# radhofan/Fairify

Measured on AMD Instinct MI355X. Metric: % partitions verified + partitions/sec on AC suite at 1/2/4/8 MI355X, higher is better.
Workload: dtype fp32

## Files before the change

fairify_amd/csrc/bindings.cpp:

```cpp
#include <hip/hip_runtime.h>
#include <pybind11/pybind11.h>
#include <pybind11/stl.h>

#include <algorithm>
#include <cmath>
#include <cstring>
#include <cstdint>
#include <stdexcept>
#include <vector>

#include "kwargs.h"
#include "runtime_host.h"

extern "C" int fa_bounds_launch(const NetDesc& net, BoundArgs args, hipStream_t stream);
extern "C" int fa_crown_phase_launch(const NetDesc& net, CrownPhaseArgs a, hipStream_t stream);
extern "C" size_t fa_crown_phase_bytes(const NetDesc& net);
extern "C" int fa_point_try_launch(const NetDesc& net, BoundArgs a, hipStream_t stream);
extern "C" int fa_forward_launch(const NetDesc& net, FwdArgs a, hipStream_t stream);
extern "C" int fa_sim_launch(const NetDesc& net, SimArgs a, hipStream_t stream);
extern "C" int fa_sim_shaped(const NetDesc& net);
extern "C" int fa_rate_launch(const NetDesc& net, RateArgs a, hipStream_t stream);
extern "C" int fa_count_enum_launch(const NetDesc& net, EnumArgs a, hipStream_t stream);
extern "C" int fa_count_rows_launch(CountArgs a, hipStream_t stream);
extern "C" int fa_count_level_launch(CountArgs a, hipStream_t stream);
// ... 213 lines not shown
  a.tau = k.f("tau", 0.f);
  a.osg = k.ptr<const int8_t>("osg");
  a.pgsum = k.ptr<const float>("pgsum");
  a.pgn = k.ptr<const float>("pgn");
  a.fpar = k.ptr<float>("fpar");
  a.fgt = k.ptr<float>("fgt");
  a.fval = k.ptr<double>("fval");
  if ((net.d.dims[0] < 64 && (a.ramask >> net.d.dims[0])) || (a.ramask && (!a.plo || !a.phi)))
    throw std::invalid_argument("beta_level: RA mask beyond the inputs or no x' box");
  return a;
}

PYBIND11_MODULE(_C, m) {
  m.doc() = "fairify_amd CDNA4 (gfx950) kernels";
  py::class_<Net>(m, "Net")
      .def(py::init<const std::vector<int>&, double>())
      .def_readonly("n_params", &Net::n_params)
      .def_readonly("total_floats", &Net::total_floats)
      .def_property_readonly("wperm_off", [](const Net& n) { return n.d.wperm_off; })
      .def_property_readonly("pack_g", [](const Net& n) { return n.d.pack_g; })
      .def_property_readonly("pack_off", [](const Net& n) { return n.d.pack_off; })
      .def_property_readonly("n_hidden", [](const Net& n) { return n.d.n_hidden; })
      .def_property_readonly("n_neurons", [](const Net& n) { return n.d.n_neurons; });

  m.def("bounds", [](const Net& net, py::kwargs kw) {
    Kw k("bounds", kw);
    const int symbolic = k.i("symbolic");
    BoundArgs a = bound_args(k, symbolic ? OUT | FORMS : OUT);
    a.symbolic = symbolic;
    a.G = k.i("G", 0);
    a.dead_out = k.ptr<uint8_t>("dead_out");
    a.fold = k.u64("fold", 0);
    a.phase_in = k.ptr<const int8_t>("phase_in");
    a.infeas = k.ptr<uint8_t>("infeas");
    ckl(fa_bounds_launch(net.d, a, finish(k)), "bounds");
  });

  m.def("crown_phase", [](const Net& net, py::kwargs kw) {
    Kw k("crown_phase", kw);
    CrownPhaseArgs a = row_args<CrownPhaseArgs>(k, OUT | FORMS | LAYERS);
    a.phase = k.ptr<const int8_t>("phase");
    a.infeas = k.ptr<const uint8_t>("infeas");
    a.split = k.need<int>("split");
    a.score = k.need<float>("score");
    a.low = k.ptr<float>("low");
    const int rc = fa_crown_phase_launch(net.d, a, finish(k));
    if (rc != 0) throw std::runtime_error("crown_phase launch failed, code " + std::to_string(rc));
  });

  m.def("relu_fits", [](const Net& net) { return fa_crown_phase_bytes(net.d) > 0; });

  m.def("crown", [](const Net& net, py::kwargs kw) {
    Kw k("crown", kw);
    const BoundArgs a = bound_args(k, OUT | FORMS | LAYERS);
    ckl(fa_crown_launch(net.d, a, finish(k)), "crown");
  });

  m.def("refine", [](const Net& net, py::kwargs kw) {
    Kw k("refine", kw);
    BoundArgs a = bound_args(k, LAYERS);
    a.phase_in = k.ptr<const int8_t>("phase_in");
    a.infeas = k.ptr<uint8_t>("infeas");
    const int rc = fa_refine_launch(net.d, a, finish(k));
    if (rc < -1) throw std::runtime_error("refine launch failed, code " + std::to_string(rc));
    return rc;
  });
  m.def("refine_crown", [](const Net& net, py::kwargs kw) {
    Kw k("refine_crown", kw);
    const BoundArgs a = bound_args(k, OUT | FORMS | LAYERS);
    const int rc = fa_refine_crown_launch(net.d, a, finish(k));
    if (rc < -1) throw std::runtime_error("refine_crown launch failed, code " + std::to_string(rc));
    return rc;
  });
  m.def("backward_bounds", [](const Net& net, py::kwargs kw) {
    Kw k("backward_bounds", kw);
    const BoundArgs a = bound_args(k, OUT | FORMS);
    const int rc = fa_backward_launch(net.d, a, finish(k));
    if (rc < -1) throw std::runtime_error("backward_bounds launch failed, code " + std::to_string(rc));
    return rc;
  });

  m.def("point_bounds", [](const Net& net, py::kwargs kw) {
    Kw k("point_bounds", kw);
    const BoundArgs a = bound_args(k, OUT, "x", "x");
    const hipStream_t stream = finish(k);
    const int rc = fa_point_try_launch(net.d, a, stream);
    if (rc < 0) ckl(-rc, "point_bounds");
    if (rc == 0) ckl(fa_bounds_launch(net.d, a, stream), "point_bounds(ibp)");
  });

  m.def("forward", [](const Net& net, uintptr_t flat, uintptr_t x, int B, uintptr_t dead, uintptr_t out,
                      uintptr_t stream) {
    FwdArgs a{};
    a.flat = P<const float>(flat);
    a.x = P<const float>(x);
    a.B = B;
    a.dead = P<const uint8_t>(dead);
    a.out = P<float>(out);
    ckl(fa_forward_launch(net.d, a, (hipStream_t)stream), "forward");
  });

  m.def("sim", [](const Net& net, py::kwargs kw) {
    Kw k("sim", kw);
    SimArgs a{};
    fill_query(a, k, "too many PA/RA dims");
    fill_samples(a, k, "too many PA/RA dims");
    a.counts = k.need<int>("counts");
    a.found = k.need<uint8_t>("found");
    a.wit_x = k.need<float>("wit_x");
    a.wit_xp = k.need<float>("wit_xp");
    a.z0 = k.ptr<float>("z0");
    a.keys = k.ptr<int>("keys");
    a.split = k.i("split");
    a.regcount = k.i("regcount");
    if (a.split < 1 || (a.split > 1 && !a.keys)) throw std::invalid_argument("sim: split > 1 needs a keys buffer");
    ckl(fa_sim_launch(net.d, a, finish(k)), "sim");
  });
  m.def("sim_shaped", [](const Net& net) { return fa_sim_shaped(net.d) != 0; });

  m.def("rate", [](const Net& net, py::kwargs kw) {
    Kw k("rate", kw);
    RateArgs a{};
    fill_query(a, k, "too many PA/RA dims");
    fill_samples(a, k, "too many PA/RA dims");
    a.E = k.i("E");
    a.flips = k.need<int>("flips");
    a.amb = k.need<int>("amb");
    a.amb_idx = k.need<int>("amb_idx");
    a.split = k.i("split");
    const int rc = fa_rate_launch(net.d, a, finish(k));
    if (rc == -3) throw std::invalid_argument("rate: shape not covered (layer > 160, inputs > 32, V > 32 or E > 32)");
    ckl(rc, "rate");
  });

  m.def("count_enum", [](const Net& net, py::kwargs kw) {
    Kw k("count_enum", kw);
    EnumArgs a{};
    a.flat = k.need<const float>("flat");
    a.lo = k.need<const float>("lo");
    a.hi = k.need<const float>("hi");
    a.L = k.i("L");
    a.V = k.i("V");
    a.npa = dims(k, "pa", a.pa_idx, FA_MAX_PA, "too many PA/RA dims");
    a.values = k.need<const int64_t>("values");
    a.Pp = k.i("Pp");
    a.pairs = k.ptr<const int64_t>("pairs");
    a.nra = dims(k, "ra", a.ra_idx, FA_MAX_RA, "too many PA/RA dims");
    a.tau = k.i("tau");
    a.E = k.i("E");
    a.max_vol = k.i("max_vol");
    a.cert = k.need<int>("cert");
    a.amb = k.need<int>("amb");
    a.amb_idx = k.need<int>("amb_idx");
    a.blocks = k.i("blocks");
    if (a.Pp > 0 && !a.pairs) throw py::type_error("count_enum() missing required keyword argument 'pairs'");
    const int rc = fa_count_enum_launch(net.d, a, finish(k));
    if (rc == -3)
      throw std::invalid_argument(
          "count_enum: shape not covered (layer > 160, inputs > 32, V > 32, E > 32 or leaf volume > 65536)");
    ckl(rc, "count_enum");
  });
  auto count_args = [](Kw& k) {
    CountArgs a{};
    a.N = k.i("N");
    a.n0 = k.i("n0");
    a.V = k.i("V");
    a.npa = dims(k, "pa", a.pa_idx, FA_MAX_PA, "too many PA/RA dims");
// ... 247 lines not shown
```

fairify_amd/csrc/crown.hip:

```cpp
#include <hip/hip_runtime.h>

#include <stdlib.h>

#include <algorithm>
#include <map>
#include <mutex>

#include "args.h"

#define FA_CROWN_MAXW 256
#define FA_CROWN_WAVES 4

__device__ __forceinline__ float fa_gam(int k, float u) {
  const float ku = (float)(k + 2) * u;
  return ku / (1.f - ku) * (1.f + 4.f * u);
}

template <int G>
__device__ __forceinline__ float fa_group_sum(float v) {
#pragma unroll
  for (int off = G / 2; off > 0; off >>= 1) v += __shfl_xor(v, off, 64);
  return v;
}

template <int G>
__global__ void __launch_bounds__(64 * FA_CROWN_WAVES) fa_crown_kernel(NetDesc net, BoundArgs a, int nparams, int WP) {
  extern __shared__ __attribute__((aligned(16))) float smem[];
  constexpr int RPW = 64 / G;
  const int tid = threadIdx.x;
  for (int l = 0; l < net.n_layers; ++l) {
    const int nin = net.dims[l], nout = net.dims[l + 1];
    const float* src = a.flat + net.w_off[l];
    float* dst = smem + net.w_off[l];
    for (int e = tid; e < nin * nout; e += 64 * FA_CROWN_WAVES) {
      const int j = e / nin, i = e - j * nin;
      dst[e] = src[(size_t)i * nout + j];
    }
    for (int e = tid; e < nout; e += 64 * FA_CROWN_WAVES) smem[net.b_off[l] + e] = a.flat[net.b_off[l] + e];
  }
  __syncthreads();
  const int lane = tid & 63;
  const int wave = tid >> 6;
  const int grp = lane / G;
  const int gl = lane % G;
  float* lam = smem + nparams + (wave * RPW + grp) * (4 * WP + 1);
  float* mu = lam + 2 * WP;
  const int L = net.n_layers;
  const int n0 = net.dims[0];
  const int N = net.n_neurons;
  const float u = net.unit;
  const int rows_per_block = FA_CROWN_WAVES * RPW;
  for (int rb = blockIdx.x * rows_per_block; rb < a.R; rb += gridDim.x * rows_per_block) {
    const int r0 = rb + wave * RPW + grp;
    const bool valid = r0 < a.R;
    const int r = valid ? r0 : a.R - 1;
    const int node = a.V > 0 ? r / a.V : r;
    const int v = a.V > 0 ? r - node * a.V : 0;
    const uint8_t* dmask = nullptr;
    if (a.dead_in) dmask = a.dead_in + (size_t)r * net.n_hidden;
    else if (a.dead_part) dmask = a.dead_part + (size_t)a.node_part[node] * net.n_hidden;
    const float* lbr = a.layer_lb + (size_t)r * N;
    const float* ubr = a.layer_ub + (size_t)r * N;
    {
      const int n = net.dims[L - 1];
      const float* W = smem + net.w_off[L - 1];
      for (int i = gl; i < n; i += G) {
        lam[i] = W[i];
        lam[WP + i] = -W[i];
      }
    }
    float c[2], err[2];
    c[0] = smem[net.b_off[L - 1]];
    c[1] = -c[0];
    err[0] = err[1] = 0.f;
    __builtin_amdgcn_wave_barrier();
    for (int l = L - 2; l >= 0; --l) {
      const int n = net.dims[l + 1];
      const int nin = net.dims[l];
      const int off = net.neuron_off[l];
      const float* W = smem + net.w_off[l];
      const float* b = smem + net.b_off[l];
      float cs[2] = {0.f, 0.f}, cm[2] = {0.f, 0.f}, er[2] = {0.f, 0.f};
      for (int j = gl; j < n; j += G) {
        const float lb = lbr[off + j], ub = ubr[off + j];
        const bool dd = ub <= 0.f || (dmask && dmask[off + j]);
        const bool act = !dd && lb >= 0.f;
        const bool unst = !dd && !act;
        const float alpha = ub > -lb ? 1.f : 0.f;
        const float s = unst ? (ub / (ub - lb)) * (1.f + 4.f * u) : 0.f;
        const float zmax = fmaxf(fabsf(lb), fabsf(ub));
        const float bj = b[j];
#pragma unroll
        for (int sg = 0; sg < 2; ++sg) {
          const float lm = lam[sg * WP + j];
          const float slope = act ? 1.f : (dd ? 0.f : (lm >= 0.f ? alpha : s));
          const float m = lm * slope;
// ... 10 lines not shown
      for (int i = gl; i < nin; i += G) {
        float acc0 = 0.f, acc1 = 0.f, mag0 = 0.f, mag1 = 0.f;
        for (int j = 0; j < n; ++j) {
          const float w = W[(size_t)j * nin + i];
          const float m0 = mu[j], m1 = mu[WP + j];
          acc0 = fmaf(w, m0, acc0);
          acc1 = fmaf(w, m1, acc1);
          mag0 = fmaf(fabsf(w), fabsf(m0), mag0);
          mag1 = fmaf(fabsf(w), fabsf(m1), mag1);
        }
        float hm;
        if (l > 0) {
          const int po = net.neuron_off[l - 1];
          hm = fmaxf(ubr[po + i], 0.f);
          if (dmask && dmask[po + i]) hm = 0.f;
        } else {
          float xl = a.lo[(size_t)node * n0 + i], xh = a.hi[(size_t)node * n0 + i];
          if (a.V > 0)
            for (int k = 0; k < a.npa; ++k)
              if (a.pa_idx[k] == i) xl = xh = a.values[v * a.npa + k];
          hm = fmaxf(fabsf(xl), fabsf(xh));
        }
        lam[i] = acc0;
        lam[WP + i] = acc1;
        er[0] += gn * mag0 * hm;
        er[1] += gn * mag1 * hm;
      }
      const float gc = fa_gam(2 * n + 1, u);
#pragma unroll
      for (int sg = 0; sg < 2; ++sg) {
        const float csum = fa_group_sum<G>(cs[sg]);
        const float cmag = fa_group_sum<G>(cm[sg]);
        const float esum = fa_group_sum<G>(er[sg]);
        const float cold = c[sg];
        c[sg] = cold + csum;
        err[sg] += esum + gc * (fabsf(cold) + cmag);
      }
      __builtin_amdgcn_wave_barrier();
    }
    int K = 4 * L + 4;
    for (int l = 0; l < L; ++l) K += 2 * net.dims[l + 1];
    const float gK = fa_gam(K, u);
    const float g0 = fa_gam(n0 + 1, u);
    const float g1 = fa_gam(1, u);
    float low[2];
#pragma unroll
    for (int sg = 0; sg < 2; ++sg) {
      float cp = 0.f, mp = 0.f;
      for (int i = gl; i < n0; i += G) {
        float xl = a.lo[(size_t)node * n0 + i], xh = a.hi[(size_t)node * n0 + i];
        if (a.V > 0)
          for (int k = 0; k < a.npa; ++k)
            if (a.pa_idx[k] == i) xl = xh = a.values[v * a.npa + k];
        const float lm = lam[sg * WP + i];
        cp += fminf(lm * xl, lm * xh);
        mp += fabsf(lm) * fmaxf(fabsf(xl), fabsf(xh));
      }
      const float conc = fa_group_sum<G>(cp) + c[sg];
      const float cmg = fa_group_sum<G>(mp) + fabsf(c[sg]);
      err[sg] *= 1.f + 2.f * gK;
      low[sg] = conc - err[sg] - g0 * cmg - g1 * fabsf(conc);
    }
    if (valid) {
      const float olb = a.out_lb[r], oub = a.out_ub[r];
      const bool useL = low[0] >= olb;
      const bool useU = -low[1] <= oub;
      for (int i = gl; i < n0; i += G) {
        if (useL) a.Lc[(size_t)r * n0 + i] = lam[i];
        if (useU) a.Uc[(size_t)r * n0 + i] = -lam[WP + i];
      }
      if (gl == 0) {
        if (useL) { a.L0[r] = c[0]; a.Le[r] = err[0]; a.out_lb[r] = low[0]; }
        if (useU) { a.U0[r] = -c[1]; a.Ue[r] = err[1]; a.out_ub[r] = -low[1]; }
      }
    }
    __builtin_amdgcn_wave_barrier();
  }
}

struct CrownCfg {
  int w_lds[FA_MAX_LAYERS];
  int b_lds[FA_MAX_LAYERS];
  int floats;
};

#ifndef FA_CROWN_WPE4
#define FA_CROWN_WPE4 3
#endif
#ifndef FA_CROWN_WPE7
#define FA_CROWN_WPE7 2
#endif
template <int TM>
__global__ void __launch_bounds__(256)
__attribute__((amdgpu_waves_per_eu(TM == 4 ? FA_CROWN_WPE4 : (TM == 7 ? FA_CROWN_WPE7 : 1)))) fa_crown_mfma_kernel(NetDesc net, BoundArgs a, CrownCfg cfg) {
  extern __shared__ __attribute__((aligned(16))) float smem[];
  const int tid = threadIdx.x;
  for (int l = 0; l < net.n_layers; ++l) {
    const int nin = net.dims[l], nout = net.dims[l + 1];
    const int tin = (nin + 15) >> 4, tout = (nout + 15) >> 4;
    const float* W = a.flat + net.w_off[l];
    float* dst = smem + cfg.w_lds[l];
    const int tot = tin * tout * 256;
    for (int e = tid; e < tot; e += 256) {
      const int i4 = e & 3, ln = (e >> 2) & 63, tt = e >> 8;
      const int t = tt % tout, ot = tt / tout;
      const int in = 16 * ot + (ln & 15), out = 16 * t + 4 * (ln >> 4) + i4;
      dst[e] = (in < nin && out < nout) ? W[(size_t)in * nout + out] : 0.f;
    }
    for (int e = tid; e < nout; e += 256) smem[cfg.b_lds[l] + e] = a.flat[net.b_off[l] + e];
  }
  __syncthreads();
  const int lane = tid & 63, col = lane & 15, grp = lane >> 4;
  const int wave = tid >> 6;
  const int L = net.n_layers;
  const int n0 = net.dims[0];
  const int N = net.n_neurons;
  const float u = net.unit;
  const int ntile = (a.R + 15) >> 4;
  for (int tile = blockIdx.x * 4 + wave; tile < ntile; tile += gridDim.x * 4) {
    const int r0 = tile * 16 + col;
    const bool valid = r0 < a.R;
    const int r = valid ? r0 : a.R - 1;
    const int node = a.V > 0 ? r / a.V : r;
    const int v = a.V > 0 ? r - node * a.V : 0;
    if (a.skip_status) {
      const int8_t st = a.skip_status[a.skip_part[node]];
      if (!__any(valid && (st == 3 || st == 4))) continue;
    }
    const uint8_t* dmask = nullptr;
    if (a.dead_in) dmask = a.dead_in + (size_t)r * net.n_hidden;
    else if (a.dead_part) dmask = a.dead_part + (size_t)a.node_part[a.part_mod ? node % a.part_mod : node] * net.n_hidden;
    const float* lbr = a.layer_lb + (size_t)r * N;
    const float* ubr = a.layer_ub + (size_t)r * N;
    float lam[2][TM][4];
    {
      const int n = net.dims[L - 1];
      const float* W = a.flat + net.w_off[L - 1];
#pragma unroll
      for (int t = 0; t < TM; ++t)
#pragma unroll
        for (int i = 0; i < 4; ++i) {
          const int j = 16 * t + 4 * grp + i;
          const float w = j < n ? W[j] : 0.f;
          lam[0][t][i] = w;
          lam[1][t][i] = -w;
        }
    }
    float c[2], err[2];
    c[0] = smem[cfg.b_lds[L - 1]];
    c[1] = -c[0];
    err[0] = err[1] = 0.f;
    for (int l = L - 2; l >= 0; --l) {
      const int n = net.dims[l + 1];
      const int nin = net.dims[l];
      const int tout = (n + 15) >> 4, tin = (nin + 15) >> 4;
      const int off = net.neuron_off[l];
      const float* b = smem + cfg.b_lds[l];
      float mu[2][TM][4];
      float cs[2] = {0.f, 0.f}, cm[2] = {0.f, 0.f}, er[2] = {0.f, 0.f};
#pragma unroll
      for (int t = 0; t < TM; ++t)
#pragma unroll
        for (int i = 0; i < 4; ++i) {
          const int j = 16 * t + 4 * grp + i;
          const bool jv = t < tout && j < n;
          const float lb = jv ? lbr[off + j] : 0.f, ub = jv ? ubr[off + j] : 0.f;
          const bool dd = !jv || ub <= 0.f || (dmask && dmask[off + j]);
          const bool act = !dd && lb >= 0.f;
          const bool unst = !dd && !act;
          const float alpha = ub > -lb ? 1.f : 0.f;
          const float sl = unst ? (ub / (ub - lb)) * (1.f + 4.f * u) : 0.f;
          const float zmax = fmaxf(fabsf(lb), fabsf(ub));
          const float bj = jv ? b[j] : 0.f;
#pragma unroll
          for (int sg = 0; sg < 2; ++sg) {
            const float lm = lam[sg][t][i];
            const float slope = act ? 1.f : (dd ? 0.f : (lm >= 0.f ? alpha : sl));
            const float m = lm * slope;
            const bool neg = unst && lm < 0.f;
            const float tt = neg ? -m * lb : 0.f;
            mu[sg][t][i] = m;
            cs[sg] += m * bj + tt;
            cm[sg] += fabsf(m * bj) + fabsf(tt);
            if (neg) er[sg] += 3.f * u * (fabsf(m) * zmax + fabsf(tt));
          }
        }
      float amu[2][TM][4];
#pragma unroll
      for (int t = 0; t < TM; ++t)
#pragma unroll
        for (int i = 0; i < 4; ++i) {
          amu[0][t][i] = fabsf(mu[0][t][i]);
          amu[1][t][i] = fabsf(mu[1][t][i]);
        }
      const float4* wb = reinterpret_cast<const float4*>(smem + cfg.w_lds[l]);
      const float gn = fa_gam(2 * n + 1, u);
#pragma unroll
      for (int ot = 0; ot < TM; ++ot) {
        if (ot >= tin) break;
        f32x4 Z0 = {0.f, 0.f, 0.f, 0.f}, Z1 = Z0, Q0 = Z0, Q1 = Z0;
#pragma unroll
        for (int t = 0; t < TM; ++t) {
          if (t >= tout) break;
          const float4 w4 = wb[(ot * tout + t) * 64 + lane];
          const float wv[4] = {w4.x, w4.y, w4.z, w4.w};
#pragma unroll
          for (int i = 0; i < 4; ++i) {
            const float aw = fabsf(wv[i]);
            Z0 = fa_mfma4(wv[i], mu[0][t][i], Z0);
            Z1 = fa_mfma4(wv[i], mu[1][t][i], Z1);
            Q0 = fa_mfma4(aw, amu[0][t][i], Q0);
            Q1 = fa_mfma4(aw, amu[1][t][i], Q1);
          }
        }
#pragma unroll
        for (int i = 0; i < 4; ++i) {
          const int in = 16 * ot + 4 * grp + i;
          float hm = 0.f;
          if (in < nin) {
            if (l > 0) {
              const int po = net.neuron_off[l - 1];
              hm = fmaxf(ubr[po + in], 0.f);
              if (dmask && dmask[po + in]) hm = 0.f;
            } else {
              float xl = a.lo[(size_t)node * n0 + in], xh = a.hi[(size_t)node * n0 + in];
              if (a.V > 0)
                for (int k = 0; k < a.npa; ++k)
                  if (a.pa_idx[k] == in) xl = xh = a.values[v * a.npa + k];
              hm = fmaxf(fabsf(xl), fabsf(xh));
            }
          }
          lam[0][ot][i] = in < nin ? Z0[i] : 0.f;
          lam[1][ot][i] = in < nin ? Z1[i] : 0.f;
          er[0] += gn * Q0[i] * hm;
          er[1] += gn * Q1[i] * hm;
        }
      }
#pragma unroll
      for (int ot = 0; ot < TM; ++ot)
        if (ot >= tin)
#pragma unroll
          for (int i = 0; i < 4; ++i) lam[0][ot][i] = lam[1][ot][i] = 0.f;
      const float gc = fa_gam(2 * n + 1, u);
#pragma unroll
      for (int sg = 0; sg < 2; ++sg) {
        float csum = cs[sg], cmag = cm[sg], esum = er[sg];
        csum += __shfl_xor(csum, 16); csum += __shfl_xor(csum, 32);
        cmag += __shfl_xor(cmag, 16); cmag += __shfl_xor(cmag, 32);
        esum += __shfl_xor(esum, 16); esum += __shfl_xor(esum, 32);
        const float cold = c[sg];
        c[sg] = cold + csum;
        err[sg] += esum + gc * (fabsf(cold) + cmag);
      }
    }
    int K = 4 * L + 4;
    for (int l = 0; l < L; ++l) K += 2 * net.dims[l + 1];
    const float gK = fa_gam(K, u);
    const float g0 = fa_gam(n0 + 1, u);
    const float g1 = fa_gam(1, u);
    float low[2];
#pragma unroll
    for (int sg = 0; sg < 2; ++sg) {
      float cp = 0.f, mp = 0.f;
#pragma unroll
      for (int t = 0; t < TM; ++t)
#pragma unroll
        for (int i = 0; i < 4; ++i) {
          const int in = 16 * t + 4 * grp + i;
          if (in >= n0) continue;
          float xl = a.lo[(size_t)node * n0 + in], xh = a.hi[(size_t)node * n0 + in];
          if (a.V > 0)
            for (int k = 0; k < a.npa; ++k)
              if (a.pa_idx[k] == in) xl = xh = a.values[v * a.npa + k];
          const float lm = lam[sg][t][i];
          cp += fminf(lm * xl, lm * xh);
          mp += fabsf(lm) * fmaxf(fabsf(xl), fabsf(xh));
        }
      cp += __shfl_xor(cp, 16); cp += __shfl_xor(cp, 32);
      mp += __shfl_xor(mp, 16); mp += __shfl_xor(mp, 32);
      const float conc = cp + c[sg];
      const float cmg = mp + fabsf(c[sg]);
      err[sg] *= 1.f + 2.f * gK;
      low[sg] = conc - err[sg] - g0 * cmg - g1 * fabsf(conc);
    }
    if (valid) {
      const float olb = a.out_lb[r], oub = a.out_ub[r];
      const bool useL = low[0] >= olb;
      const bool useU = -low[1] <= oub;
#pragma unroll
      for (int t = 0; t < TM; ++t)
#pragma unroll
        for (int i = 0; i < 4; ++i) {
          const int in = 16 * t + 4 * grp + i;
          if (in >= n0) continue;
          if (useL) a.Lc[(size_t)r * n0 + in] = lam[0][t][i];
          if (useU) a.Uc[(size_t)r * n0 + in] = -lam[1][t][i];
        }
      if (grp == 0) {
        if (useL) { a.L0[r] = c[0]; a.Le[r] = err[0]; a.out_lb[r] = low[0]; }
        if (useU) { a.U0[r] = -c[1]; a.Ue[r] = err[1]; a.out_ub[r] = -low[1]; }
      }
    }
  }
}

namespace {
typedef void (*CrownMfmaKernel)(NetDesc, BoundArgs, CrownCfg);
CrownMfmaKernel select_crown_mfma(int TM) {
  if (TM <= 1) return fa_crown_mfma_kernel<1>;
  if (TM <= 2) return fa_crown_mfma_kernel<2>;
  if (TM <= 4) return fa_crown_mfma_kernel<4>;
  if (TM <= 7) return fa_crown_mfma_kernel<7>;
  return nullptr;
}

int crown_cus() {
  static int cus = 0;
  static std::once_flag once;
  std::call_once(once, [] {
    int dev = 0;
    if (hipGetDevice(&dev) != hipSuccess ||
        hipDeviceGetAttribute(&cus, hipDeviceAttributeMultiprocessorCount, dev) != hipSuccess || cus <= 0)
      cus = 256;
  });
  return cus;
}

int crown_mfma_try(const NetDesc& net, const BoundArgs& a, hipStream_t stream) {
  static const bool off = [] {
    const char* e = getenv("FAIRIFY_CROWN_MFMA");
    return e && e[0] == '0';
  }();
  if (off) return 0;
  int TM = 1;
  for (int l = 0; l <= net.n_layers; ++l) TM = std::max(TM, (net.dims[l] + 15) / 16);
  CrownMfmaKernel k = select_crown_mfma(TM);
  if (!k) return 0;
  CrownCfg cfg{};
  int offs = 0;
  for (int l = 0; l < net.n_layers; ++l) {
    cfg.w_lds[l] = offs;
    offs += ((net.dims[l] + 15) / 16) * ((net.dims[l + 1] + 15) / 16) * 256;
  }
  for (int l = 0; l < net.n_layers; ++l) {
    cfg.b_lds[l] = offs;
    offs += net.dims[l + 1];
  }
  cfg.floats = (offs + 3) & ~3;
  const size_t bytes = (size_t)cfg.floats * sizeof(float);
  if (bytes > 150 * 1024) return 0;
  static std::mutex mu;
  static std::map<std::pair<const void*, size_t>, int> occ;
  int per_cu = 0;
  {
    std::lock_guard<std::mutex> g(mu);
    const auto key = std::make_pair((const void*)k, bytes);
    auto it = occ.find(key);
    if (it == occ.end()) {
      if (!fa_lds_ok(bytes)) return -4;
      if (hipOccupancyMaxActiveBlocksPerMultiprocessor(&per_cu, k, 256, bytes) != hipSuccess || per_cu <= 0) per_cu = 1;
      occ[key] = per_cu;
    } else {
      per_cu = it->second;
    }
  }
  const long long tiles = (a.R + 15) / 16;
  long long blocks = (tiles + 3) / 4;
  const long long cap = (long long)crown_cus() * per_cu;
  if (blocks > cap) blocks = cap;
  hipLaunchKernelGGL(k, dim3((unsigned)blocks), dim3(256), bytes, stream, net, a, cfg);
  const hipError_t e = hipGetLastError();
  return e == hipSuccess ? 1 : -(int)e;
}
}

extern "C" int fa_crown_launch(const NetDesc& net, BoundArgs a, hipStream_t stream) {
  if (a.R <= 0) return 0;
  if (!a.layer_lb || !a.layer_ub || !a.Lc || !a.Uc) return -2;
  {
    const int rc = crown_mfma_try(net, a, stream);
    if (rc == 1) return 0;
    if (rc < 0) return -3;
  }
  int wmax = 1;
  for (int l = 0; l <= net.n_layers; ++l) {
    if (net.dims[l] > FA_CROWN_MAXW) return -1;
    if (l > 0) wmax = std::max(wmax, net.dims[l]);
  }
  int G = 4;
  while (G < wmax && G < 64) G *= 2;
  const int WP = (std::max(wmax, net.dims[0]) + 3) & ~3;
  int nparams = 0;
  for (int l = 0; l < net.n_layers; ++l) nparams = net.b_off[l] + net.dims[l + 1];
  const int rows_per_block = FA_CROWN_WAVES * (64 / G);
  const size_t bytes = ((size_t)nparams + (size_t)rows_per_block * (4 * WP + 1)) * sizeof(float);
  if (bytes > 160 * 1024) return -1;
  typedef void (*K)(NetDesc, BoundArgs, int, int);
  K k = G == 4 ? fa_crown_kernel<4> : G == 8 ? fa_crown_kernel<8> : G == 16 ? fa_crown_kernel<16>
      : G == 32 ? fa_crown_kernel<32> : fa_crown_kernel<64>;
  if (!fa_lds_ok(bytes)) return -3;
  const int blocks = (int)std::min<long long>(((long long)a.R + rows_per_block - 1) / rows_per_block, 256LL * 8);
  hipLaunchKernelGGL(k, dim3(blocks), dim3(64 * FA_CROWN_WAVES), bytes, stream, net, a, nparams, WP);
  return (int)hipGetLastError();
}

FA_LDS_REGISTER(FA_LDS_K(fa_crown_mfma_kernel<1>), FA_LDS_K(fa_crown_mfma_kernel<2>), FA_LDS_K(fa_crown_mfma_kernel<4>),
                FA_LDS_K(fa_crown_mfma_kernel<7>), FA_LDS_K(fa_crown_kernel<4>), FA_LDS_K(fa_crown_kernel<8>),
                FA_LDS_K(fa_crown_kernel<16>), FA_LDS_K(fa_crown_kernel<32>), FA_LDS_K(fa_crown_kernel<64>));
```

fairify_amd/csrc/points.hip:

```cpp
#include <hip/hip_runtime.h>

#include <algorithm>
#include <map>
#include <mutex>

#include "pointfwd.h"

template <int TM>
__global__ void __launch_bounds__(FA_THREADS) __attribute__((amdgpu_waves_per_eu(TM == 7 ? 2 : 1))) fa_point_kernel(NetDesc net, BoundArgs a, PointCfg cfg) {
  extern __shared__ __attribute__((aligned(16))) float smem[];
  const int tid = threadIdx.x;
  {
    const float4* src = reinterpret_cast<const float4*>(a.flat + net.wperm_off);
    float4* dst = reinterpret_cast<float4*>(smem);
    for (int e = tid; e < (net.wperm_floats >> 2); e += FA_THREADS) dst[e] = src[e];
    for (int l = 0; l < net.n_layers; ++l) {
      const int n_out = net.dims[l + 1];
      const float* b = a.flat + net.wperm_off + cfg.b_lds[l];
      for (int j = tid; j < ((n_out + 15) & ~15); j += FA_THREADS) smem[cfg.bp_lds[l] + j] = j < n_out ? b[j] : 0.f;
    }
  }
  __syncthreads();
  const int lane = tid & 63, col = lane & 15, grp = lane >> 4;
  const int wave = tid >> 6, nw = FA_THREADS / 64;
  const int n0 = net.dims[0];
  const int tin0 = (n0 + 15) >> 4;
  const float g0 = net.g_fwd[0];
  const int ntile = (a.R + 15) >> 4;
  for (int tile = blockIdx.x * nw + wave; tile < ntile; tile += gridDim.x * nw) {
    const int p0 = tile * 16;
    const int p = p0 + col;
    if (a.row_open && !__any(p < a.R && a.row_open[p % a.open_mod])) continue;
    float HA[TM][4], EA[TM][4], HB[TM][4], EB[TM][4];
#pragma unroll
    for (int t = 0; t < TM; ++t) {
      if (t >= tin0) break;
#pragma unroll
      for (int i = 0; i < 4; ++i) {
        const int k = 16 * t + 4 * grp + i;
        const float x = (k < n0 && p < a.R) ? a.lo[(size_t)p * n0 + k] : 0.f;
        HA[t][i] = x;
        EA[t][i] = g0 * fabsf(x);
      }
    }
    for (int l = 0; l < net.n_layers; ++l) {
      if (l & 1) fa_point_layer<TM>(net, a, cfg, smem, l, p0, lane, HB, EB, HA, EA);
      else fa_point_layer<TM>(net, a, cfg, smem, l, p0, lane, HA, EA, HB, EB);
    }
  }
}

namespace {
typedef void (*PointKernel)(NetDesc, BoundArgs, PointCfg);

PointKernel select_point(int TM) {
  if (TM <= 1) return fa_point_kernel<1>;
  if (TM <= 2) return fa_point_kernel<2>;
  if (TM <= 4) return fa_point_kernel<4>;
  if (TM <= 7) return fa_point_kernel<7>;
  if (TM <= 10) return fa_point_kernel<10>;
  return nullptr;
}

int point_cus() {
  static int cus = 0;
  static std::once_flag once;
  std::call_once(once, [] {
    int dev = 0;
    if (hipGetDevice(&dev) != hipSuccess ||
        hipDeviceGetAttribute(&cus, hipDeviceAttributeMultiprocessorCount, dev) != hipSuccess || cus <= 0)
      cus = 256;
  });
  return cus;
}
}

extern "C" int fa_point_try_launch(const NetDesc& net, BoundArgs a, hipStream_t stream) {
  if (a.R <= 0) return 1;
  int TM = 1;
  for (int l = 0; l <= net.n_layers; ++l) TM = std::max(TM, (net.dims[l] + 15) / 16);
  PointKernel k = select_point(TM);
  if (!k) return 0;
  PointCfg cfg{};
  int off = 0;
  for (int l = 0; l < net.n_layers; ++l) {
    cfg.w_lds[l] = off;
    off += ((net.dims[l] + 15) / 16) * ((net.dims[l + 1] + 15) / 16) * 256;
  }
  for (int l = 0; l < net.n_layers; ++l) {
    cfg.b_lds[l] = off;
    off += net.dims[l + 1];
  }
  if (((off + 3) & ~3) != net.wperm_floats) return -1;
  if ((size_t)net.wperm_floats * sizeof(float) > 150 * 1024) return 0;
// ... 34 lines not shown
```

Baseline: 268,100.

## Specialize CROWN MFMA kernel on compile-time network shapes and dead-mask presence

Adds templated CROWN kernels specialized for known network shapes (AC suite architectures), unrolling layers at compile time with constexpr offsets, cached input-box registers, and a no-mask variant that drops dead-neuron loads. It also copies pre-permuted weights into LDS with float4 when available, and lets the point-bounds kernel exit early when no rows in the block are open. The aim is to cut register pressure, index arithmetic and redundant global loads in the hot backward pass, at the cost of many more kernel instantiations and longer compile time. Floating-point contraction is disabled and some arithmetic is rewritten as explicit fmaf, which keeps the rounding-error bounds sound.

```diff
diff --git a/fairify_amd/csrc/bindings.cpp b/fairify_amd/csrc/bindings.cpp
--- a/fairify_amd/csrc/bindings.cpp
+++ b/fairify_amd/csrc/bindings.cpp
@@ -319,7 +319,10 @@
 
   m.def("point_bounds", [](const Net& net, py::kwargs kw) {
     Kw k("point_bounds", kw);
-    const BoundArgs a = bound_args(k, OUT, "x", "x");
+    BoundArgs a = bound_args(k, OUT, "x", "x");
+    a.row_open = k.ptr<const uint8_t>("row_open");
+    a.open_mod = k.i("open_mod", 0);
+    if (a.row_open && a.open_mod <= 0) throw std::invalid_argument("point_bounds: row_open needs open_mod > 0");
     const hipStream_t stream = finish(k);
     const int rc = fa_point_try_launch(net.d, a, stream);
     if (rc < 0) ckl(-rc, "point_bounds");
diff --git a/fairify_amd/csrc/crown.hip b/fairify_amd/csrc/crown.hip
--- a/fairify_amd/csrc/crown.hip
+++ b/fairify_amd/csrc/crown.hip
@@ -12,6 +12,7 @@
 #define FA_CROWN_WAVES 4
 
 __device__ __forceinline__ float fa_gam(int k, float u) {
+#pragma clang fp contract(off)
   const float ku = (float)(k + 2) * u;
   return ku / (1.f - ku) * (1.f + 4.f * u);
 }
@@ -188,7 +189,203 @@
   int w_lds[FA_MAX_LAYERS];
   int b_lds[FA_MAX_LAYERS];
   int floats;
+  int wfloats;
+  int wcopy;
 };
+
+template <class S>
+struct CrownLay {
+  __host__ __device__ static constexpr int tiles(int l) { return (S::dim(l) + 15) / 16; }
+  __host__ __device__ static constexpr int w_lds(int l) {
+    int o = 0;
+    for (int k = 0; k < l; ++k) o += tiles(k) * tiles(k + 1) * 256;
+    return o;
+  }
+  __host__ __device__ static constexpr int b_lds(int l) {
+    int o = w_lds(S::L);
+    for (int k = 0; k < l; ++k) o += S::dim(k + 1);
+    return o;
+  }
+  __host__ __device__ static constexpr int neuron_off(int l) {
+    int o = 0;
+    for (int k = 0; k < l; ++k) o += S::dim(k + 1);
+    return o;
+  }
+  __host__ __device__ static constexpr int conc_terms() {
+    int K = 4 * S::L + 4;
+    for (int l = 0; l < S::L; ++l) K += 2 * S::dim(l + 1);
+    return K;
+  }
+};
+
+__device__ __forceinline__ void fa_crown_box(const BoundArgs& a, int node, int v, int n0, int in, float& xl, float& xh) {
+  xl = a.lo[(size_t)node * n0 + in];
+  xh = a.hi[(size_t)node * n0 + in];
+  if (a.V > 0)
+    for (int k = 0; k < a.npa; ++k)
+      if (a.pa_idx[k] == in) xl = xh = a.values[v * a.npa + k];
+}
+
+template <int TM, class S, int LC, int TB, bool MASK>
+__device__ __forceinline__ void fa_crown_layer(const NetDesc& net, const BoundArgs& a, const CrownCfg& cfg,
+                                               const float* smem, int lrt, int lane, int grp, int node, int v,
+                                               const float* lbr, const float* ubr, const uint8_t* dmask, float u,
+                                               const float (&bxl)[TB][4], const float (&bxh)[TB][4],
+                                               float (&lam)[2][TM][4], float (&c)[2], float (&err)[2]) {
+#pragma clang fp contract(off)
+  constexpr bool SH = S::L > 0;
+  using Y = CrownLay<S>;
+  constexpr int TO = SH ? Y::tiles(LC + 1) : TM;
+  constexpr int TI = SH ? Y::tiles(LC) : TM;
+  const int l = SH ? LC : lrt;
+  const int n = SH ? S::dim(LC + 1) : net.dims[l + 1];
+  const int nin = SH ? S::dim(LC) : net.dims[l];
+  const int tout = (n + 15) >> 4, tin = (nin + 15) >> 4;
+  const int off = SH ? Y::neuron_off(LC) : net.neuron_off[l];
+  const float* b = smem + (SH ? Y::b_lds(LC) : cfg.b_lds[l]);
+  const int n0 = SH ? S::dim(0) : net.dims[0];
+  float mu[2][TM][4];
+  float cs[2] = {0.f, 0.f}, cm[2] = {0.f, 0.f}, er[2] = {0.f, 0.f};
+#pragma unroll
+  for (int t = 0; t < TO; ++t)
+#pragma unroll
+    for (int i = 0; i < 4; ++i) {
+      const int j = 16 * t + 4 * grp + i;
+      const bool jv = t < tout && j < n;
+      const int jc = jv ? j : 0;
+      const float lbv = lbr[off + jc], ubv = ubr[off + jc], bv = b[jc];
+      bool dmv = false;
+      if constexpr (MASK) dmv = dmask[off + jc] != 0;
+      const float lb = jv ? lbv : 0.f, ub = jv ? ubv : 0.f;
+      const bool dd = !jv | (ub <= 0.f) | dmv;
+      const bool act = !dd && lb >= 0.f;
+      const bool unst = !dd && !act;
+      const float alpha = ub > -lb ? 1.f : 0.f;
+      float chord = 0.f;
+      if (TM > 1 || __any(unst)) chord = (ub / (ub - lb)) * (1.f + 4.f * u);
+      const float sl = unst ? chord : 0.f;
+      const float zmax = fmaxf(fabsf(lb), fabsf(ub));
+      const float bj = jv ? bv : 0.f;
+#pragma unroll
+      for (int sg = 0; sg < 2; ++sg) {
+        const float lm = lam[sg][t][i];
+        const float slope = act ? 1.f : (dd ? 0.f : (lm >= 0.f ? alpha : sl));
+        const float m = lm * slope;
+        const bool neg = unst && lm < 0.f;
+        const float tt = neg ? -m * lb : 0.f;
+        mu[sg][t][i] = m;
+        cs[sg] += fmaf(m, bj, tt);
+        cm[sg] += fabsf(m * bj) + fabsf(tt);
+        if (neg) er[sg] = fmaf(3.f * u, fmaf(fabsf(m), zmax, fabsf(tt)), er[sg]);
+      }
+    }
+  constexpr bool AMU = !SH || TI == 1;
+  float amu[2][AMU ? TM : 1][4];
+  if constexpr (AMU) {
+#pragma unroll
+    for (int t = 0; t < TO; ++t)
+#pragma unroll
+      for (int i = 0; i < 4; ++i) {
+        amu[0][t][i] = fabsf(mu[0][t][i]);
+        amu[1][t][i] = fabsf(mu[1][t][i]);
+      }
+  }
+  const float4* wb = reinterpret_cast<const float4*>(smem + (SH ? Y::w_lds(LC) : cfg.w_lds[l]));
+  const float gn = fa_gam(2 * n + 1, u);
+#pragma unroll
+  for (int ot = 0; ot < TI; ++ot) {
+    if constexpr (!SH) {
+      if (ot >= tin) break;
+    } else {
+      __builtin_amdgcn_sched_barrier(0);
+    }
+    f32x4 Z0 = {0.f, 0.f, 0.f, 0.f}, Z1 = Z0, Q0 = Z0, Q1 = Z0;
+#pragma unroll
+    for (int t = 0; t < TO; ++t) {
+      if constexpr (!SH) {
+        if (t >= tout) break;
+      }
+      const float4 w4 = wb[(ot * tout + t) * 64 + lane];
+      const float wv[4] = {w4.x, w4.y, w4.z, w4.w};
+#pragma unroll
+      for (int i = 0; i < 4; ++i) {
+        const float aw = fabsf(wv[i]);
+        Z0 = fa_mfma4(wv[i], mu[0][t][i], Z0);
+        Z1 = fa_mfma4(wv[i], mu[1][t][i], Z1);
+        float am0, am1;
+        if constexpr (AMU) {
+          am0 = amu[0][t][i];
+          am1 = amu[1][t][i];
+        } else {
+          float m0 = mu[0][t][i], m1 = mu[1][t][i];
+          asm volatile("" : "+v"(m0), "+v"(m1));
+          am0 = fabsf(m0);
+          am1 = fabsf(m1);
+        }
+        Q0 = fa_mfma4(aw, am0, Q0);
+        Q1 = fa_mfma4(aw, am1, Q1);
+      }
+    }
+#pragma unroll
+    for (int i = 0; i < 4; ++i) {
+      const int in = 16 * ot + 4 * grp + i;
+      float hm = 0.f;
+      if (SH ? LC > 0 : l > 0) {
+        const int po = SH ? Y::neuron_off(LC > 0 ? LC - 1 : 0) : net.neuron_off[l - 1];
+        const int ic = in < nin ? in : 0;
+        const float hu = fmaxf(ubr[po + ic], 0.f);
+        bool hd = false;
+        if constexpr (MASK) hd = dmask[po + ic] != 0;
+        hm = ((in >= nin) | hd) ? 0.f : hu;
+      } else if (in < nin) {
+        {
+          float xl, xh;
+          if constexpr (SH && TM < 7) {
+            xl = bxl[ot < TB ? ot : 0][i];
+            xh = bxh[ot < TB ? ot : 0][i];
+          } else {
+            fa_crown_box(a, node, v, n0, in, xl, xh);
+          }
+          hm = fmaxf(fabsf(xl), fabsf(xh));
+        }
+      }
+      lam[0][ot][i] = in < nin ? Z0[i] : 0.f;
+      lam[1][ot][i] = in < nin ? Z1[i] : 0.f;
+      er[0] = fmaf(gn * Q0[i], hm, er[0]);
+      er[1] = fmaf(gn * Q1[i], hm, er[1]);
+    }
+  }
+  if constexpr (!SH) {
+#pragma unroll
+    for (int ot = 0; ot < TM; ++ot)
+      if (ot >= tin)
+#pragma unroll
+        for (int i = 0; i < 4; ++i) lam[0][ot][i] = lam[1][ot][i] = 0.f;
+  }
+  const float gc = fa_gam(2 * n + 1, u);
+#pragma unroll
+  for (int sg = 0; sg < 2; ++sg) {
+    float csum = cs[sg], cmag = cm[sg], esum = er[sg];
+    csum += __shfl_xor(csum, 16); csum += __shfl_xor(csum, 32);
+    cmag += __shfl_xor(cmag, 16); cmag += __shfl_xor(cmag, 32);
+    esum += __shfl_xor(esum, 16); esum += __shfl_xor(esum, 32);
+    const float cold = c[sg];
+    c[sg] = cold + csum;
+    err[sg] += fmaf(gc, fabsf(cold) + cmag, esum);
+  }
+}
+
+template <int TM, class S, int TB, bool MASK, int... IS>
+__device__ __forceinline__ void fa_crown_layers_c(std::integer_sequence<int, IS...>, const NetDesc& net,
+                                                  const BoundArgs& a, const CrownCfg& cfg, const float* smem, int lane,
+                                                  int grp, int node, int v, const float* lbr, const float* ubr,
+                                                  const uint8_t* dmask, float u, const float (&bxl)[TB][4],
+                                                  const float (&bxh)[TB][4], float (&lam)[2][TM][4], float (&c)[2],
+                                                  float (&err)[2]) {
+  (fa_crown_layer<TM, S, S::L - 2 - IS, TB, MASK>(net, a, cfg, smem, 0, lane, grp, node, v, lbr, ubr, dmask, u, bxl, bxh,
+                                            lam, c, err),
+   ...);
+}
 
 #ifndef FA_CROWN_WPE4
 #define FA_CROWN_WPE4 3
@@ -196,32 +393,58 @@
 #ifndef FA_CROWN_WPE7
 #define FA_CROWN_WPE7 2
 #endif
-template <int TM>
+template <int TM, class S = FaShapeAny, bool MASK = true>
 __global__ void __launch_bounds__(256)
-__attribute__((amdgpu_waves_per_eu(TM == 4 ? FA_CROWN_WPE4 : (TM == 7 ? FA_CROWN_WPE7 : 1)))) fa_crown_mfma_kernel(NetDesc net, BoundArgs a, CrownCfg cfg) {
+__attribute__((amdgpu_waves_per_eu(TM == 4 ? FA_CROWN_WPE4 : (TM == 7 ? FA_CROWN_WPE7 : (S::L > 0 ? 3 : 1))))) fa_crown_mfma_kernel(NetDesc net, BoundArgs a, CrownCfg cfg) {
+#pragma clang fp contract(off)
   extern __shared__ __attribute__((aligned(16))) float smem[];
+  constexpr bool SH = S::L > 0;
+  using Y = CrownLay<S>;
+  constexpr int TB = SH ? Y::tiles(0) : 1;
+  constexpr int TL = SH ? Y::tiles(SH ? S::L - 1 : 0) : TM;
   const int tid = threadIdx.x;
+  if (cfg.wcopy) {
+    const float4* src = reinterpret_cast<const float4*>(a.flat + net.wback_off);
+    float4* dst = reinterpret_cast<float4*>(smem);
+    for (int e = tid; e < (cfg.wfloats >> 2); e += 256) dst[e] = src[e];
+  }
   for (int l = 0; l < net.n_layers; ++l) {
     const int nin = net.dims[l], nout = net.dims[l + 1];
-    const int tin = (nin + 15) >> 4, tout = (nout + 15) >> 4;
-    const float* W = a.flat + net.w_off[l];
-    float* dst = smem + cfg.w_lds[l];
-    const int tot = tin * tout * 256;
-    for (int e = tid; e < tot; e += 256) {
-      const int i4 = e & 3, ln = (e >> 2) & 63, tt = e >> 8;
-      const int t = tt % tout, ot = tt / tout;
-      const int in = 16 * ot + (ln & 15), out = 16 * t + 4 * (ln >> 4) + i4;
-      dst[e] = (in < nin && out < nout) ? W[(size_t)in * nout + out] : 0.f;
+    if (!cfg.wcopy) {
+      const int tin = (nin + 15) >> 4, tout = (nout + 15) >> 4;
+      const float* W = a.flat + net.w_off[l];
+      float* dst = smem + cfg.w_lds[l];
+      const int tot = tin * tout * 256;
+      for (int e = tid; e < tot; e += 256) {
+        const int i4 = e & 3, ln = (e >> 2) & 63, tt = e >> 8;
+        const int t = tt % tout, ot = tt / tout;
+        const int in = 16 * ot + (ln & 15), out = 16 * t + 4 * (ln >> 4) + i4;
+        dst[e] = (in < nin && out < nout) ? W[(size_t)in * nout + out] : 0.f;
+      }
     }
     for (int e = tid; e < nout; e += 256) smem[cfg.b_lds[l] + e] = a.flat[net.b_off[l] + e];
   }
   __syncthreads();
   const int lane = tid & 63, col = lane & 15, grp = lane >> 4;
   const int wave = tid >> 6;
-  const int L = net.n_layers;
-  const int n0 = net.dims[0];
-  const int N = net.n_neurons;
-  const float u = net.unit;
+  const int L = SH ? S::L : net.n_layers;
+  const int n0 = SH ? S::dim(0) : net.dims[0];
+  const int N = SH ? Y::neuron_off(S::L) : net.n_neurons;
+  const float u = SH ? 0x1p-24f : net.unit;
+  int pslot[TB][4];
+  if constexpr (SH) {
+#pragma unroll
+    for (int t = 0; t < TB; ++t)
+#pragma unroll
+      for (int i = 0; i < 4; ++i) {
+        const int in = 16 * t + 4 * grp + i;
+        int s = -1;
+        if (a.V > 0)
+          for (int k = 0; k < a.npa; ++k)
+            if (a.pa_idx[k] == in) s = k;
+        pslot[t][i] = s;
+      }
+  }
   const int ntile = (a.R + 15) >> 4;
   for (int tile = blockIdx.x * 4 + wave; tile < ntile; tile += gridDim.x * 4) {
     const int r0 = tile * 16 + col;
@@ -234,16 +457,35 @@
       if (!__any(valid && (st == 3 || st == 4))) continue;
     }
     const uint8_t* dmask = nullptr;
-    if (a.dead_in) dmask = a.dead_in + (size_t)r * net.n_hidden;
-    else if (a.dead_part) dmask = a.dead_part + (size_t)a.node_part[a.part_mod ? node % a.part_mod : node] * net.n_hidden;
+    if constexpr (MASK) {
+      if (a.dead_in) dmask = a.dead_in + (size_t)r * net.n_hidden;
+      else dmask = a.dead_part + (size_t)a.node_part[a.part_mod ? node % a.part_mod : node] * net.n_hidden;
+    }
     const float* lbr = a.layer_lb + (size_t)r * N;
     const float* ubr = a.layer_ub + (size_t)r * N;
+    float bxl[TB][4], bxh[TB][4];
+    if constexpr (SH) {
+#pragma unroll
+      for (int t = 0; t < TB; ++t)
+#pragma unroll
+        for (int i = 0; i < 4; ++i) {
+          const int in = 16 * t + 4 * grp + i;
+          float xl = 0.f, xh = 0.f;
+          if (in < n0) {
+            xl = a.lo[(size_t)node * n0 + in];
+            xh = a.hi[(size_t)node * n0 + in];
+            if (pslot[t][i] >= 0) xl = xh = a.values[v * a.npa + pslot[t][i]];
+          }
+          bxl[t][i] = xl;
+          bxh[t][i] = xh;
+        }
+    }
     float lam[2][TM][4];
     {
-      const int n = net.dims[L - 1];
+      const int n = SH ? S::dim(SH ? S::L - 1 : 0) : net.dims[L - 1];
       const float* W = a.flat + net.w_off[L - 1];
 #pragma unroll
-      for (int t = 0; t < TM; ++t)
+      for (int t = 0; t < TL; ++t)
 #pragma unroll
         for (int i = 0; i < 4; ++i) {
           const int j = 16 * t + 4 * grp + i;
@@ -253,131 +495,44 @@
         }
     }
     float c[2], err[2];
-    c[0] = smem[cfg.b_lds[L - 1]];
+    c[0] = smem[SH ? Y::b_lds(SH ? S::L - 1 : 0) : cfg.b_lds[L - 1]];
     c[1] = -c[0];
     err[0] = err[1] = 0.f;
-    for (int l = L - 2; l >= 0; --l) {
-      const int n = net.dims[l + 1];
-      const int nin = net.dims[l];
-      const int tout = (n + 15) >> 4, tin = (nin + 15) >> 4;
-      const int off = net.neuron_off[l];
-      const float* b = smem + cfg.b_lds[l];
-      float mu[2][TM][4];
-      float cs[2] = {0.f, 0.f}, cm[2] = {0.f, 0.f}, er[2] = {0.f, 0.f};
-#pragma unroll
-      for (int t = 0; t < TM; ++t)
-#pragma unroll
-        for (int i = 0; i < 4; ++i) {
-          const int j = 16 * t + 4 * grp + i;
-          const bool jv = t < tout && j < n;
-          const float lb = jv ? lbr[off + j] : 0.f, ub = jv ? ubr[off + j] : 0.f;
-          const bool dd = !jv || ub <= 0.f || (dmask && dmask[off + j]);
-          const bool act = !dd && lb >= 0.f;
-          const bool unst = !dd && !act;
-          const float alpha = ub > -lb ? 1.f : 0.f;
-          const float sl = unst ? (ub / (ub - lb)) * (1.f + 4.f * u) : 0.f;
-          const float zmax = fmaxf(fabsf(lb), fabsf(ub));
-          const float bj = jv ? b[j] : 0.f;
-#pragma unroll
-          for (int sg = 0; sg < 2; ++sg) {
-            const float lm = lam[sg][t][i];
-            const float slope = act ? 1.f : (dd ? 0.f : (lm >= 0.f ? alpha : sl));
-            const float m = lm * slope;
-            const bool neg = unst && lm < 0.f;
-            const float tt = neg ? -m * lb : 0.f;
-            mu[sg][t][i] = m;
-            cs[sg] += m * bj + tt;
-            cm[sg] += fabsf(m * bj) + fabsf(tt);
-            if (neg) er[sg] += 3.f * u * (fabsf(m) * zmax + fabsf(tt));
-          }
-        }
-      float amu[2][TM][4];
-#pragma unroll
-      for (int t = 0; t < TM; ++t)
-#pragma unroll
-        for (int i = 0; i < 4; ++i) {
-          amu[0][t][i] = fabsf(mu[0][t][i]);
-          amu[1][t][i] = fabsf(mu[1][t][i]);
-        }
-      const float4* wb = reinterpret_cast<const float4*>(smem + cfg.w_lds[l]);
-      const float gn = fa_gam(2 * n + 1, u);
-#pragma unroll
-      for (int ot = 0; ot < TM; ++ot) {
-        if (ot >= tin) break;
-        f32x4 Z0 = {0.f, 0.f, 0.f, 0.f}, Z1 = Z0, Q0 = Z0, Q1 = Z0;
-#pragma unroll
-        for (int t = 0; t < TM; ++t) {
-          if (t >= tout) break;
-          const float4 w4 = wb[(ot * tout + t) * 64 + lane];
-          const float wv[4] = {w4.x, w4.y, w4.z, w4.w};
-#pragma unroll
-          for (int i = 0; i < 4; ++i) {
-            const float aw = fabsf(wv[i]);
-            Z0 = fa_mfma4(wv[i], mu[0][t][i], Z0);
-            Z1 = fa_mfma4(wv[i], mu[1][t][i], Z1);
-            Q0 = fa_mfma4(aw, amu[0][t][i], Q0);
-            Q1 = fa_mfma4(aw, amu[1][t][i], Q1);
-          }
-        }
-#pragma unroll
-        for (int i = 0; i < 4; ++i) {
-          const int in = 16 * ot + 4 * grp + i;
-          float hm = 0.f;
-          if (in < nin) {
-            if (l > 0) {
-              const int po = net.neuron_off[l - 1];
-              hm = fmaxf(ubr[po + in], 0.f);
-              if (dmask && dmask[po + in]) hm = 0.f;
-            } else {
-              float xl = a.lo[(size_t)node * n0 + in], xh = a.hi[(size_t)node * n0 + in];
-              if (a.V > 0)
-                for (int k = 0; k < a.npa; ++k)
-                  if (a.pa_idx[k] == in) xl = xh = a.values[v * a.npa + k];
-              hm = fmaxf(fabsf(xl), fabsf(xh));
-            }
-          }
-          lam[0][ot][i] = in < nin ? Z0[i] : 0.f;
-          lam[1][ot][i] = in < nin ? Z1[i] : 0.f;
-          er[0] += gn * Q0[i] * hm;
-          er[1] += gn * Q1[i] * hm;
-        }
-      }
-#pragma unroll
-      for (int ot = 0; ot < TM; ++ot)
-        if (ot >= tin)
-#pragma unroll
-          for (int i = 0; i < 4; ++i) lam[0][ot][i] = lam[1][ot][i] = 0.f;
-      const float gc = fa_gam(2 * n + 1, u);
-#pragma unroll
-      for (int sg = 0; sg < 2; ++sg) {
-        float csum = cs[sg], cmag = cm[sg], esum = er[sg];
-        csum += __shfl_xor(csum, 16); csum += __shfl_xor(csum, 32);
-        cmag += __shfl_xor(cmag, 16); cmag += __shfl_xor(cmag, 32);
-        esum += __shfl_xor(esum, 16); esum += __shfl_xor(esum, 32);
-        const float cold = c[sg];
-        c[sg] = cold + csum;
-        err[sg] += esum + gc * (fabsf(cold) + cmag);
-      }
+    if constexpr (SH) {
+      fa_crown_layers_c<TM, S, TB, MASK>(std::make_integer_sequence<int, S::L - 1>{}, net, a, cfg, smem, lane, grp, node, v,
+                                   lbr, ubr, dmask, u, bxl, bxh, lam, c, err);
+    } else {
+      for (int l = L - 2; l >= 0; --l)
+        fa_crown_layer<TM, S, 0, TB, MASK>(net, a, cfg, smem, l, lane, grp, node, v, lbr, ubr, dmask, u, bxl, bxh, lam, c,
+                                     err);
     }
     int K = 4 * L + 4;
-    for (int l = 0; l < L; ++l) K += 2 * net.dims[l + 1];
+    if constexpr (SH) {
+      K = Y::conc_terms();
+    } else {
+      for (int l = 0; l < L; ++l) K += 2 * net.dims[l + 1];
+    }
     const float gK = fa_gam(K, u);
     const float g0 = fa_gam(n0 + 1, u);
     const float g1 = fa_gam(1, u);
+    constexpr int TC = SH ? TB : TM;
     float low[2];
 #pragma unroll
     for (int sg = 0; sg < 2; ++sg) {
       float cp = 0.f, mp = 0.f;
 #pragma unroll
-      for (int t = 0; t < TM; ++t)
+      for (int t = 0; t < TC; ++t)
 #pragma unroll
         for (int i = 0; i < 4; ++i) {
           const int in = 16 * t + 4 * grp + i;
           if (in >= n0) continue;
-          float xl = a.lo[(size_t)node * n0 + in], xh = a.hi[(size_t)node * n0 + in];
-          if (a.V > 0)
-            for (int k = 0; k < a.npa; ++k)
-              if (a.pa_idx[k] == in) xl = xh = a.values[v * a.npa + k];
+          float xl, xh;
+          if constexpr (SH && TM < 7) {
+            xl = bxl[t][i];
+            xh = bxh[t][i];
+          } else {
+            fa_crown_box(a, node, v, n0, in, xl, xh);
+          }
           const float lm = lam[sg][t][i];
           cp += fminf(lm * xl, lm * xh);
           mp += fabsf(lm) * fmaxf(fabsf(xl), fabsf(xh));
@@ -386,15 +541,17 @@
       mp += __shfl_xor(mp, 16); mp += __shfl_xor(mp, 32);
       const float conc = cp + c[sg];
       const float cmg = mp + fabsf(c[sg]);
-      err[sg] *= 1.f + 2.f * gK;
-      low[sg] = conc - err[sg] - g0 * cmg - g1 * fabsf(conc);
+      const float eo = err[sg], ef = 1.f + 2.f * gK;
+      err[sg] = eo * ef;
+      const float ce = fmaf(-ef, eo, conc);
+      low[sg] = sg == 0 ? fmaf(-g1, fabsf(conc), fmaf(-g0, cmg, ce)) : (ce - g0 * cmg) - g1 * fabsf(conc);
     }
     if (valid) {
       const float olb = a.out_lb[r], oub = a.out_ub[r];
       const bool useL = low[0] >= olb;
       const bool useU = -low[1] <= oub;
 #pragma unroll
-      for (int t = 0; t < TM; ++t)
+      for (int t = 0; t < TC; ++t)
 #pragma unroll
         for (int i = 0; i < 4; ++i) {
           const int in = 16 * t + 4 * grp + i;
@@ -412,11 +569,45 @@
 
 namespace {
 typedef void (*CrownMfmaKernel)(NetDesc, BoundArgs, CrownCfg);
-CrownMfmaKernel select_crown_mfma(int TM) {
-  if (TM <= 1) return fa_crown_mfma_kernel<1>;
-  if (TM <= 2) return fa_crown_mfma_kernel<2>;
-  if (TM <= 4) return fa_crown_mfma_kernel<4>;
-  if (TM <= 7) return fa_crown_mfma_kernel<7>;
+CrownMfmaKernel select_crown_mfma(int TM, bool mask) {
+  if (TM <= 1) return mask ? fa_crown_mfma_kernel<1> : fa_crown_mfma_kernel<1, FaShapeAny, false>;
+  if (TM <= 2) return mask ? fa_crown_mfma_kernel<2> : fa_crown_mfma_kernel<2, FaShapeAny, false>;
+  if (TM <= 4) return mask ? fa_crown_mfma_kernel<4> : fa_crown_mfma_kernel<4, FaShapeAny, false>;
+  if (TM <= 7) return mask ? fa_crown_mfma_kernel<7> : fa_crown_mfma_kernel<7, FaShapeAny, false>;
+  return nullptr;
+}
+
+struct ShapedCrown {
+  int tm;
+  std::vector<int> dims;
+  CrownMfmaKernel k[2];
+};
+template <int TM, int... D>
+ShapedCrown shaped_crown() {
+  return {TM, {D...}, {fa_crown_mfma_kernel<TM, FaShape<D...>, false>, fa_crown_mfma_kernel<TM, FaShape<D...>, true>}};
+}
+
+CrownMfmaKernel select_crown_shaped(const NetDesc& net, int TM, bool mask) {
+  const char* e = getenv("FAIRIFY_CROWN_SHAPED");
+  if (e && *e == '0') return nullptr;
+  if (net.unit != 0x1p-24f) return nullptr;
+  static const std::vector<ShapedCrown> v = {
+      shaped_crown<7, 13, 100, 100, 1>(),
+      shaped_crown<7, 13, 100, 1>(),
+      shaped_crown<4, 13, 64, 64, 1>(),
+      shaped_crown<4, 13, 50, 1>(),
+      shaped_crown<1, 13, 5, 5, 1>(),
+      shaped_crown<1, 13, 16, 8, 1>(),
+      shaped_crown<1, 13, 12, 12, 1>(),
+      shaped_crown<1, 13, 3, 3, 3, 3, 1>(),
+  };
+  const int tmb = TM <= 1 ? 1 : TM <= 2 ? 2 : TM <= 4 ? 4 : 7;
+  for (const auto& s : v) {
+    if (s.tm != tmb || (int)s.dims.size() != net.n_layers + 1) continue;
+    bool same = true;
+    for (int l = 0; l <= net.n_layers && same; ++l) same = s.dims[l] == net.dims[l];
+    if (same) return s.k[mask ? 1 : 0];
+  }
   return nullptr;
 }
 
@@ -440,14 +631,18 @@
   if (off) return 0;
   int TM = 1;
   for (int l = 0; l <= net.n_layers; ++l) TM = std::max(TM, (net.dims[l] + 15) / 16);
-  CrownMfmaKernel k = select_crown_mfma(TM);
+  const bool mask = a.dead_in || a.dead_part;
+  CrownMfmaKernel k = select_crown_mfma(TM, mask);
   if (!k) return 0;
+  if (const CrownMfmaKernel ks = select_crown_shaped(net, TM, mask)) k = ks;
   CrownCfg cfg{};
   int offs = 0;
   for (int l = 0; l < net.n_layers; ++l) {
     cfg.w_lds[l] = offs;
     offs += ((net.dims[l] + 15) / 16) * ((net.dims[l + 1] + 15) / 16) * 256;
   }
+  cfg.wfloats = offs;
+  cfg.wcopy = net.wback_floats == offs && (net.wback_off & 3) == 0;
   for (int l = 0; l < net.n_layers; ++l) {
     cfg.b_lds[l] = offs;
     offs += net.dims[l + 1];
@@ -513,3 +708,11 @@
 FA_LDS_REGISTER(FA_LDS_K(fa_crown_mfma_kernel<1>), FA_LDS_K(fa_crown_mfma_kernel<2>), FA_LDS_K(fa_crown_mfma_kernel<4>),
                 FA_LDS_K(fa_crown_mfma_kernel<7>), FA_LDS_K(fa_crown_kernel<4>), FA_LDS_K(fa_crown_kernel<8>),
                 FA_LDS_K(fa_crown_kernel<16>), FA_LDS_K(fa_crown_kernel<32>), FA_LDS_K(fa_crown_kernel<64>));
+#define FA_CROWN_LDS(TM, ...)                                         \
+  FA_LDS_K((fa_crown_mfma_kernel<TM, FaShape<__VA_ARGS__>, true>)), \
+      FA_LDS_K((fa_crown_mfma_kernel<TM, FaShape<__VA_ARGS__>, false>))
+FA_LDS_REGISTER(FA_LDS_K((fa_crown_mfma_kernel<1, FaShapeAny, false>)), FA_LDS_K((fa_crown_mfma_kernel<2, FaShapeAny, false>)),
+                FA_LDS_K((fa_crown_mfma_kernel<4, FaShapeAny, false>)), FA_LDS_K((fa_crown_mfma_kernel<7, FaShapeAny, false>)));
+FA_LDS_REGISTER(FA_CROWN_LDS(7, 13, 100, 100, 1), FA_CROWN_LDS(7, 13, 100, 1), FA_CROWN_LDS(4, 13, 64, 64, 1),
+                FA_CROWN_LDS(4, 13, 50, 1), FA_CROWN_LDS(1, 13, 5, 5, 1),
+                FA_CROWN_LDS(1, 13, 16, 8, 1), FA_CROWN_LDS(1, 13, 12, 12, 1), FA_CROWN_LDS(1, 13, 3, 3, 3, 3, 1));
diff --git a/fairify_amd/csrc/points.hip b/fairify_amd/csrc/points.hip
--- a/fairify_amd/csrc/points.hip
+++ b/fairify_amd/csrc/points.hip
@@ -10,6 +10,16 @@
 __global__ void __launch_bounds__(FA_THREADS) __attribute__((amdgpu_waves_per_eu(TM == 7 ? 2 : 1))) fa_point_kernel(NetDesc net, BoundArgs a, PointCfg cfg) {
   extern __shared__ __attribute__((aligned(16))) float smem[];
   const int tid = threadIdx.x;
+  if (a.row_open) {
+    const int nw = FA_THREADS / 64;
+    const int ntile = (a.R + 15) >> 4;
+    int any = 0;
+    for (int tile = blockIdx.x * nw + (tid >> 6); tile < ntile; tile += gridDim.x * nw) {
+      const int p = tile * 16 + (tid & 15);
+      any |= p < a.R && a.row_open[p % a.open_mod];
+    }
+    if (!__syncthreads_or(any)) return;
+  }
   {
     const float4* src = reinterpret_cast<const float4*>(a.flat + net.wperm_off);
     float4* dst = reinterpret_cast<float4*>(smem);
```

After: 277,100, median of 6. +3.3%, better.
